# Klaudiusz321/raytracing-engine-in-c

Measured on AMD Instinct MI355X. Metric: Mrays/s (and RK4 steps/s) per GPU + per node; max |Δhit| vs CPU ref, higher is better.
Workload: dtype f64

## Files before the change

include/bhrt_api.h:

```cpp
#ifndef BHRT_API_H
#define BHRT_API_H

#include "bhrt_types.h"

#ifdef __cplusplus
extern "C" {
#endif

#define BLACKHOLE_API_VERSION_MAJOR 0
#define BLACKHOLE_API_VERSION_MINOR 1
#define BLACKHOLE_API_VERSION_PATCH 0

#define BH_PI 3.14159265358979323846
#define BH_EPSILON 1.0e-10
#define BH_TWO_PI 6.28318530717958647692

typedef enum {
    BH_SUCCESS = 0,
    BH_ERROR_INVALID_PARAMETER = -1,
    BH_ERROR_MEMORY_ALLOCATION = -2,
    BH_ERROR_INITIALIZATION = -3,
    BH_ERROR_SIMULATION = -4
} BHErrorCode;

// ... 311 lines not shown
                           const bhrt_frame_soa* device_out, void* hip_stream);

int bhrt_trace_rays(const Ray* rays, int n, const BlackHoleParams* blackhole,
                    const AccretionDiskParams* disk, const SimulationConfig* config,
                    IntegrationMethod method, int flags, const bhrt_frame_soa* host_out);

#define BHRT_PATHS_MAX_POSITIONS 65536

typedef struct {
    Vector3D* xyz;
    float*    xyz32;
    int32_t*  count;
} bhrt_paths;

int bhrt_trace_paths_device(const Ray* device_rays, int n, const BlackHoleParams* blackhole,
                            const AccretionDiskParams* disk, const SimulationConfig* config,
                            IntegrationMethod method, int max_positions, int every,
                            const bhrt_paths* device_paths, const bhrt_frame_soa* device_hits,
                            void* hip_stream);

int bhrt_trace_paths(const Ray* rays, int n, const BlackHoleParams* blackhole,
                     const AccretionDiskParams* disk, const SimulationConfig* config,
                     IntegrationMethod method, int max_positions, int every,
                     const bhrt_paths* host_paths, const bhrt_frame_soa* host_hits);

int bhrt_check_rkf45_accept(const double* err, const double* scale, const double* tol, int n,
                            int* out, void* hip_stream);

int bhrt_check_disk_hit(const double* p, const double* d, const double* nrm, int n, double in_sq,
                        double out_sq, int* out, void* hip_stream);

int bhrt_check_seg_len(const double* x, int n, double* out, void* hip_stream);

int bhrt_get_stats(bhrt_stats* out, int reset);

int bhrt_device_count(void);

void bhrt_set_refill_threshold(int lanes);

int bhrt_set_claim_order(const int* d_order, int n);

int bhrt_update_particles_steps(ParticleSystem* system, const BlackHoleParams* blackhole,
                                const SimulationConfig* config, int steps, double* kernel_ms);

const char* bhrt_last_error(void);

#ifdef __cplusplus
}
#endif
#endif
```

raytracing-engine-in-c_amd/csrc/bhrt_kernel.h:

```cpp
#ifndef BHRT_KERNEL_H
#define BHRT_KERNEL_H

#include "../../include/bhrt_api.h"

#ifdef __cplusplus
extern "C" {
#endif

enum { BHRT_SRC_RAYS = 0, BHRT_SRC_CAMERA = 1 };
enum { BHRT_NUM_COUNTERS = 5 };
enum { BHRT_MAX_QUEUE_BITS = 5, BHRT_QUEUE_STRIDE_MAX = 64 };
enum { BHRT_INIT_FIELDS = 21 };
enum { BHRT_INIT_FIELDS_CAMERA = 8 };

typedef struct {
    double M, rs, two_m;
    double rs_x1_5, rs_x1_05, rs_x2_5, rs_x5, rs_x15, rs_eps;
    double h_2_5, h_5, h_15, h_far;
    double h_lo[4], h_hi[4];
    double max_dist, tol;
    double disk_in, disk_out, disk_tscale;
    double disk_in_sq, disk_out_sq;
    int max_steps;
    int method;
    int has_disk;
    int flags;
    int spin0;
    int far_bounded;
    double rot_vmax;
    int accept_all;
} bhrt_scene_k;

typedef struct {
    double fwd[3], right[3], up[3];
    double plane_w, plane_h;
    double off_x, off_y;
    int width, height;
    bhrt_rows rows;
    double inv_width, inv_block;
    double pos[3];
    double r0, th0, ph0;
    double st_cp, st_sp, ct, ct_cp, ct_sp, st, neg_sp, cp, r_st;
    double g_tt, g_rr, g_hh;
    double p0[3];
    double sp;
    double s_r0, c_r0;
    int use_approx;
    int st_tiny;
    int tile_w_log2, tile_h_log2, tiles_per_row;
    double inv_tiles_per_row;
    int ntiles, tile_stride;
} bhrt_camera_k;

#ifndef BHRT_FUSE_ALL
#define BHRT_FUSE_ALL 1
#endif
#define BHRT_COLOUR_IN_TRACE(method, has_disk, spin)                                        \
    (BHRT_FUSE_ALL ||                                                                       \
     ((has_disk) && ((method) == INTEGRATOR_RKF45 || ((method) == INTEGRATOR_RK4 && (spin)))))

typedef struct {
    bhrt_scene_k sc;
    int src;
// ... 142 lines not shown
```

raytracing-engine-in-c_amd/csrc/geodesic.hip:

```cpp
#include <hip/hip_runtime.h>

#include <atomic>

#include "bhrt_kernel.h"

#pragma clang fp contract(fast)

namespace {

constexpr double kEps = 1.0e-10;
constexpr double kTwoPi = 6.28318530717958647692;

using Scene = bhrt_scene_k;

struct Counters {
    unsigned rays = 0, iters = 0, full = 0, far_ = 0, kerr = 0;
    bool huge = false;
};

__device__ __forceinline__ double rcp_nr(double b) {
    const double y = __builtin_amdgcn_rcp(b);
    const double e = __builtin_fma(-b, y, 1.0);
    return __builtin_fma(y, __builtin_fma(e, e, e), y);
}
__device__ __forceinline__ double div_nr(double a, double , double yb) { return a * yb; }

__device__ __forceinline__ double fmac_k(double a, double b, double c) {
    double r;
    asm("v_fma_f64 %0, %1, %2, %3" : "=v"(r) : "v"(a), "v"(b), "s"(c));
    return r;
}

__device__ __forceinline__ double max_raw(double a, double b) {
    double r;
    asm("v_max_f64 %0, %1, %2" : "=v"(r) : "v"(a), "s"(b));
    return r;
}
__device__ __forceinline__ double max_abs_raw(double a, double b) {
    double r;
    asm("v_max_f64 %0, |%1|, |%2|" : "=v"(r) : "v"(a), "v"(b));
    return r;
}

__device__ __attribute__((noinline)) void sincos_ocml(double x, double* s, double* c) {
    sincos(x, s, c);
}

__device__ __forceinline__ void bhrt_sincos(double x, double* so, double* co,
                                            Counters* hc = nullptr) {
    if (!(fabs(x) < 1048576.0)) {
        if (!hc) {
            sincos_ocml(x, so, co);
            return;
        }
        if (fabs(x) <= 1.79769313486231570815e+308) hc->huge = true;
    }
    constexpr double kTwoOverPi = 6.36619772367581382433e-01;
    constexpr double P1 = 1.57079632679489655800e+00;
    constexpr double P2 = 6.12323399573676603587e-17;
    constexpr double P3 = -1.49738490485916983e-33;
    const double n = rint(x * kTwoOverPi);
    const double r1 = __builtin_fma(-n, P1, x);
    const double p2 = n * P2;
    const double p2e = __builtin_fma(n, P2, -p2);
    const double hi = r1 - p2;
    const double t = hi - r1;
    const double e = (r1 - (hi - t)) - (p2 + t);
    const double lo = __builtin_fma(-n, P3, e - p2e);
    const double r = hi + lo;
    const double y = (hi - r) + lo;
    constexpr double S1 = -1.66666666666666324348e-01, S2 = 8.33333333332248946124e-03,
                     S3 = -1.98412698298579493134e-04, S4 = 2.75573137070700676789e-06,
                     S5 = -2.50507602534068634195e-08, S6 = 1.58969099521155010221e-10;
    constexpr double C1 = 4.16666666666666019037e-02, C2 = -1.38888888888741095749e-03,
                     C3 = 2.48015872894767294178e-05, C4 = -2.75573143513906633035e-07,
                     C5 = 2.08757232129817482790e-09, C6 = -1.13596475577881948265e-11;
    const double z = r * r, w = z * z;
    const double rs_ = fmac_k(z, fmac_k(z, S4, S3), S2) + z * w * fmac_k(z, S6, S5);
    const double v = z * r;
    const double s = r - ((z * (0.5 * y - v * rs_) - y) - v * S1);
    const double rc = z * fmac_k(z, fmac_k(z, C3, C2), C1) +
                      w * w * fmac_k(z, fmac_k(z, C6, C5), C4);
    const double hz = 0.5 * z, ww = 1.0 - hz;
    const double c = ww + (((1.0 - ww) - hz) + (z * rc - r * y));
    const int q = (int)n;
    double ss = (q & 1) ? c : s;
    double cc = (q & 1) ? s : c;
    *so = (q & 2) ? -ss : ss;
// ... 79 lines not shown
        st = (st >= 0.0) ? 0.01 : -0.01;
        st2 = st * st;
    }
    const double term2 = r * y[4] * y[4];
    const double term3 = r * st2 * y[5] * y[5];
    const double n4 = -2.0 * y[3] * y[4];
    const double n5a = -2.0 * y[3] * y[5];
    const double n5b = 2.0 * y[4] * y[5] * ct;
    const double sc4 = st * ct * y[5] * y[5];
    if (r < 1.0e150) {
        const double yr = rcp_nr(r);
        const double term1 = -(sc.M * yr) * yr;
        d[3] = term1 + term2 + term3;
        d[4] = div_nr(n4, r, yr) + sc4;
        d[5] = div_nr(n5a, r, yr) - div_nr(n5b, st, rcp_nr(st));
    } else {
        const double f = 1.0 - sc.rs / r;
        const double term1 = -sc.M / (rsq * f) * f;
        d[3] = term1 + term2 + term3;
        d[4] = n4 / r + sc4;
        d[5] = n5a / r - n5b / st;
    }
}

template <bool BOUNDED = false>
__device__ __forceinline__ void repair_clamp(double (&d)[6]) {
#pragma unroll
    for (int i = BOUNDED ? 3 : 0; i < 6; i++)
        if (!isfinite(d[i])) d[i] = 0.0;
#pragma unroll
    for (int i = 3; i < 6; i++) d[i] = fmin(fmax(d[i], -10.0), 10.0);
}

#ifndef BHRT_COUNT_STAGES
#define BHRT_COUNT_STAGES 0
#endif
template <bool SPIN0, bool FAR, bool HUGE>
__device__ __forceinline__ void rhs(const double (&y)[6], double (&d)[6], const Scene& sc,
                                    bool far_ok, Counters& n, Trig1& tr, bool first) {
    d[0] = y[3];
    d[1] = y[4];
    d[2] = y[5];
    if (FAR && far_ok && y[0] > sc.rs_x15) {
        d[3] = 0.0;
        d[4] = 0.0;
        d[5] = y[5] * (sc.two_m / (y[0] * y[0]));
        n.far_++;
        return;
    }
    if (SPIN0) {
        double st, ct;
        if (first) {
            st = tr.s;
            ct = tr.c;
        } else {
            shift_or_eval(tr.a, tr.s, tr.c, y[1], st, ct, HUGE ? nullptr : &n);
        }
        if ((FAR && HUGE) || BHRT_COUNT_STAGES) n.full++;
        const double rc = max_raw(y[0], sc.rs_x1_5);
        const double w = rcp_nr(rc * st);
        const double yr = st * w, ys = rc * w;
        const double u = st * y[5];
        const double f3 = rc * __builtin_fma(u, u, y[4] * y[4]);
        d[3] = __builtin_fma(-(sc.M * yr), yr, f3);
        const double p = y[3] * yr;
        d[4] = __builtin_fma(p * -2.0, y[4], u * (ct * y[5]));
        d[5] = (y[5] * -2.0) * __builtin_fma(y[4], ct * ys, p);
        const int plain = (int)(!HUGE ? true : rc < 1.0e150) & (int)(fabs(d[3]) <= 10.0) &
                          (int)(fabs(d[4]) <= 10.0) & (int)(fabs(d[5]) <= 10.0) &
                          (int)(fabs(st) >= 0.01);
        if (__builtin_expect(plain, 1)) return;
        accel_literal(y, d, sc, st, ct);
        repair_clamp<!HUGE>(d);
        return;
    }
    d[3] = 0.0;
    d[4] = 0.0;
    d[5] = 0.0;
    if ((FAR && HUGE) || BHRT_COUNT_STAGES) n.kerr++;
    const int plain = (int)(fabs(d[3]) <= 10.0) & (int)(fabs(d[4]) <= 10.0) &
                      (int)(fabs(d[5]) <= 10.0);
    if (plain) return;
    repair_clamp<!HUGE>(d);
}

template <int METHOD, bool FAR, bool HUGE>
constexpr bool repair_at_refill() {
    return (METHOD == INTEGRATOR_RK4 || METHOD == INTEGRATOR_RKF45) && !HUGE;
}

template <bool SPIN0, bool FAR>
constexpr bool zero_accel() {
    return !SPIN0 && !FAR;
}

template <int METHOD, bool SPIN0, bool FAR, bool HUGE>
constexpr bool hoist_sums() {
    return METHOD == INTEGRATOR_RKF45 && zero_accel<SPIN0, FAR>() &&
           repair_at_refill<METHOD, FAR, HUGE>();
}

template <int METHOD, bool SPIN0, bool FAR, bool HUGE>
constexpr bool rotation_trig() {
    return zero_accel<SPIN0, FAR>() && repair_at_refill<METHOD, FAR, HUGE>() &&
           (METHOD == INTEGRATOR_RK4 || METHOD == INTEGRATOR_RKF45);
}

__device__ __forceinline__ double rk4_acc(double acc, double k) { return acc + 2.0 * k; }
constexpr double kC1 = 25.0 / 216.0, kC3 = 1408.0 / 2565.0, kC4 = 2197.0 / 4104.0,
                 kC5 = -1.0 / 5.0;
constexpr double kD1 = 16.0 / 135.0, kD3 = 6656.0 / 12825.0, kD4 = 28561.0 / 56430.0,
                 kD5 = -9.0 / 50.0, kD6 = 2.0 / 55.0;
__device__ __forceinline__ double rkf45_sum4(double k1, double k3, double k4, double k5) {
    return kC1 * k1 + kC3 * k3 + kC4 * k4 + kC5 * k5;
}
__device__ __forceinline__ double rkf45_sum5(double k1, double k3, double k4, double k5,
                                             double k6) {
    return kD1 * k1 + kD3 * k3 + kD4 * k4 + kD5 * k5 + kD6 * k6;
}

template <bool SPIN0, bool FAR, bool HUGE, bool HS = false>
__device__ __forceinline__ void rk4_step(double (&y)[6], double h, double h6, const Scene& sc,
                                         bool far_ok, Counters& n, Trig1& tr,
                                         const double* zs = nullptr) {
    constexpr bool Z = zero_accel<SPIN0, FAR>();
    double k[6], acc[6], yt[6];
    const double hh = 0.5 * h;
    rhs<SPIN0, FAR, HUGE>(y, k, sc, far_ok, n, tr, true);
#pragma unroll
    for (int i = 0; i < 6; i++) {
        acc[i] = k[i];
        yt[i] = (Z && i >= 3) ? y[i] : y[i] + hh * k[i];
    }
    rhs<SPIN0, FAR, HUGE>(yt, k, sc, far_ok, n, tr, false);
#pragma unroll
    for (int i = 0; i < 6; i++) {
        acc[i] = rk4_acc(acc[i], k[i]);
        yt[i] = (Z && i >= 3) ? y[i] : y[i] + hh * k[i];
    }
    rhs<SPIN0, FAR, HUGE>(yt, k, sc, far_ok, n, tr, false);
#pragma unroll
    for (int i = 0; i < 6; i++) {
        acc[i] = rk4_acc(acc[i], k[i]);
        yt[i] = (Z && i >= 3) ? y[i] : y[i] + h * k[i];
    }
    rhs<SPIN0, FAR, HUGE>(yt, k, sc, far_ok, n, tr, false);
#pragma unroll
    for (int i = 0; i < 6; i++) {
        if (HS && i < 3)
            y[i] = __builtin_fma(h6, zs[i], y[i]);
        else if (!(Z && i >= 3))
            y[i] = __builtin_fma(h6, acc[i] + k[i], y[i]);
    }
}

template <bool FAST, int NC = 6>
__device__ __forceinline__ bool rkf45_accept(const double (&err)[6], const double (&scale)[6],
                                             double tol) {
    const bool tol_normal = tol >= 2.2250738585072014e-308 && tol <= 1.79769313486231570815e+308;
    if (FAST && tol >= 0x1p-900 && tol <= 0x1p300) {
        const double lo = tol * (1.0 - 0x1p-40), hi = tol * (1.0 + 0x1p-40);
        bool all_pass = true;
#pragma unroll
        for (int i = 0; i < NC; i++) all_pass &= err[i] <= lo * scale[i];
        if (__builtin_expect(all_pass, 1)) return true;
        double near_max = 0.0;
        bool over = false;
#pragma unroll
        for (int i = 0; i < NC; i++) {
            const bool pass = err[i] <= lo * scale[i];
            const bool fail = err[i] > hi * scale[i];
            over |= fail;
            if (__builtin_expect(!pass && !fail, 0)) near_max = fmax(near_max, err[i] / scale[i]);
// ... 364 lines not shown
__device__ __forceinline__ HSel hsel_of(const Scene& sc) {
    return HSel{opaque<V>(sc.h_far), opaque<V>(sc.h_15), opaque<V>(sc.h_5), opaque<V>(sc.h_2_5),
                opaque<false>(0x1p100)};
}

template <bool ANCHOR = true>
__device__ __forceinline__ void state_repair(Ray_& R, Counters* hc) {
    if (__builtin_expect(
            !isfinite(((R.y[0] + R.y[1]) + (R.y[2] + R.y[3])) + (R.y[4] + R.y[5])), 0)) {
#pragma unroll
        for (int i = 0; i < 6; i++)
            if (!isfinite(R.y[i])) R.y[i] = (i < 4) ? 1.0 : 0.0;
        if (ANCHOR) trig_anchor(R, hc);
    }
}

__device__ __forceinline__ bool state_within(const Ray_& R, double bound) {
    const double m = fmax(fmax(fmax(fabs(R.y[0]), fabs(R.y[1])), fmax(fabs(R.y[2]), fabs(R.y[3]))),
                          fmax(fabs(R.y[4]), fabs(R.y[5])));
    return m <= bound;
}

template <int METHOD, bool SPIN0, bool FAR, bool HUGE>
constexpr bool hcache() {
    return (METHOD == INTEGRATOR_RK4 && !HUGE) ||
           rotation_trig<METHOD, SPIN0, FAR, HUGE>();
}

template <int METHOD, bool SPIN0, bool FAR, bool HUGE>
constexpr bool h6cache() {
    return METHOD == INTEGRATOR_RK4 && rotation_trig<METHOD, SPIN0, FAR, HUGE>();
}

template <int METHOD, bool DISK, bool SPIN0, bool FAR, bool HUGE, bool ACC = false>
__device__ __forceinline__ int ray_iterate(Ray_& R, const Scene& sc, Counters& n,
                                           const HSel hs) {
    Counters* const hc = HUGE ? nullptr : &n;
    if (!repair_at_refill<METHOD, FAR, HUGE>()) state_repair(R, hc);
    const double r = R.y[1];
    double h, h6 = 0.0;
    if constexpr (hcache<METHOD, SPIN0, FAR, HUGE>()) {
        if (__builtin_expect(!(r >= R.h_lo && r < R.h_hi), 0)) {
            int k = 0;
            k = (r < sc.rs_x15) ? 1 : k;
            k = (r < sc.rs_x5) ? 2 : k;
            k = (r < sc.rs_x2_5) ? 3 : k;
            R.h = k == 0 ? hs.far_ : (k == 1 ? hs.r15 : (k == 2 ? hs.r5 : hs.r2_5));
            R.h_lo = sc.h_lo[k];
            R.h_hi = sc.h_hi[k];
            if constexpr (rotation_trig<METHOD, SPIN0, FAR, HUGE>()) {
                double d;
                if (METHOD == INTEGRATOR_RK4) {
                    double a = R.y[5];
                    a = rk4_acc(a, R.y[5]);
                    a = rk4_acc(a, R.y[5]);
                    R.h6 = R.h * (1.0 / 6.0);
                    d = R.h6 * (a + R.y[5]);
                } else {
                    d = R.h * R.zs[5];
                }
                rotation_coeffs(d, R.cd_sd, R.cd_cm1);
            }
        }
        asm volatile("" : "+v"(R.h));
        h = R.h;
        if constexpr (h6cache<METHOD, SPIN0, FAR, HUGE>()) {
            asm volatile("" : "+v"(R.h6));
            h6 = R.h6;
        }
// ... 14 lines not shown
    } else if (METHOD == INTEGRATOR_RKF45) {
        moved = rkf45_attempt<SPIN0, FAR, HUGE, HS, ACC>(R.y, h, sc, R.far_ok, n, tr, R.zs);
    } else {
        moved = false;
    }
    double x, y, z;
    if (moved) {
        if (SPIN0) trig_advance(tr.a, R.y[1], R.s1, R.c1, hc);
        if constexpr (rotation_trig<METHOD, SPIN0, FAR, HUGE>()) {
            const double s0 = R.s2, c0 = R.c2;
            R.s2 = __builtin_fma(c0, R.cd_sd, __builtin_fma(s0, R.cd_cm1, s0));
            R.c2 = __builtin_fma(-s0, R.cd_sd, __builtin_fma(c0, R.cd_cm1, c0));
        } else {
            trig_advance(a2, R.y[2], R.s2, R.c2, hc);
        }
        if (!zero_accel<SPIN0, FAR>()) trig_advance(a3, R.y[3], R.s3, R.c3, hc);
    }
    sph2cart_t(R.y[1], R.s2, R.c2, R.s3, R.c3, x, y, z);
    const double ox = R.px, oy = R.py, oz = R.pz;
    R.dist += seg_len(x - ox, y - oy, z - oz);
    R.px = x;
    R.py = y;
    R.pz = z;
    R.k++;
    if constexpr (!DISK) {
        if (R.y[1] <= sc.rs_x1_05) return T_HORIZON;
        if (R.dist >= sc.max_dist) return T_MAXDIST;
        if (!moved) {
            R.k = sc.max_steps;
            return T_MAXSTEPS;
        }
        return R.k >= sc.max_steps ? T_MAXSTEPS : T_NONE;
    } else {
        int term = (R.k >= sc.max_steps) ? T_MAXSTEPS : T_NONE;
        term = (R.dist >= sc.max_dist) ? T_MAXDIST : term;
        term = (R.y[1] <= sc.rs_x1_05) ? T_HORIZON : term;
        double qx, qy, qz, num, den;
        if (disk_cand(R, ox, oy, oz, sc, hs.big, num, den) & (R.k < sc.max_steps)) {
            if (disk_decide(R, num, den, sc, qx, qy, qz)) {
                R.px = qx;
                R.py = qy;
                R.pz = qz;
                const double ux = qx - ox, uy = qy - oy, uz = qz - oz;
                R.dist += sqrt_nr((ux * ux + uy * uy) + uz * uz);
                term = T_DISK;
            }
        }
        if (!moved && term == T_NONE) {
            if (R.k + 1 < sc.max_steps && (x != ox || y != oy || z != oz) &&
                disk_hit(R, x, y, z, sc, hs.big, qx, qy, qz)) {
                R.px = qx;
                R.py = qy;
                R.pz = qz;
                R.k++;
                R.dist += len3(qx - x, qy - y, qz - z);
                return T_DISK;
            }
            R.k = sc.max_steps;
            return T_MAXSTEPS;
        }
        return term;
    }
}

__device__ __forceinline__ void store_hit(const bhrt_frame_soa& s, int i, const Ray_& R,
                                          int term, const Scene& sc) {
    int result, steps;
    double hx, hy, hz, tdil, sx = 0.0, sy = 0.0, sz = 0.0;
    if (term == T_DISK) {
        result = RAY_DISK;
        steps = R.k;
        hx = R.px;
        hy = R.py;
        hz = R.pz;
        tdil = 1.0 / sqrt(1.0 - sc.rs / len3(R.px, R.py, R.pz));
    } else {
        result = term == T_HORIZON ? RAY_HORIZON
                                   : (term == T_MAXDIST ? RAY_MAX_DISTANCE : RAY_MAX_STEPS);
        steps = term == T_MAXSTEPS ? R.k : R.k - 1;
// ... 286 lines not shown
template <int METHOD, bool DISK, bool SPIN0, bool FAR, int INL, bool ACC = false>
constexpr int trace_launch_waves() {
    return c3_camera<METHOD, DISK, SPIN0, FAR, false, INL>() ? 2 : ACC ? BHRT_ACC_LAUNCH_WAVES : 0;}
constexpr int BHRT_TRACE_WAVES_PER_BLOCK = 4;

__device__ __forceinline__ unsigned queue_ray(unsigned qbits, unsigned q, unsigned j) {
    return ((j >> 6) << (6u + qbits)) | (q << 6) | (j & 63u);
}
__device__ __forceinline__ unsigned queue_size(unsigned ntotal, unsigned qbits, unsigned q) {
    const unsigned nb = ntotal >> 6, last = nb & ((1u << qbits) - 1u);
    return (((nb >> qbits) + (q < last ? 1u : 0u)) << 6) + (q == last ? (ntotal & 63u) : 0u);
}
#define BHRT_TRACE_BOUNDS __attribute__((amdgpu_flat_work_group_size(1, 256), \
                                         amdgpu_waves_per_eu(trace_waves_k<METHOD, DISK, SPIN0, FAR, HUGE, INL, ACC>() > 0 ? trace_waves_k<METHOD, DISK, SPIN0, FAR, HUGE, INL, ACC>() : 1)))

#ifndef BHRT_WAVE_STAMPS
#define BHRT_WAVE_STAMPS 0
#endif
#if BHRT_WAVE_STAMPS
constexpr int kStampSlots = 64, kStampWaves = 8192, kStampWords = 8;
__device__ unsigned long long g_stamps[kStampSlots * kStampWaves * kStampWords];
#endif

#ifndef BHRT_UNROLL_ZA
#define BHRT_UNROLL_ZA 16
#endif
#ifndef BHRT_UNROLL_A0
#define BHRT_UNROLL_A0 4
#endif
template <int METHOD, bool SPIN0>
constexpr bool uniform_trip() {
    return BHRT_UNIFORM_TRIP == 1 ||
           (BHRT_UNIFORM_TRIP == 2 && METHOD == INTEGRATOR_RK4 && SPIN0);
}
template <int METHOD, bool SPIN0, bool FAR, bool HUGE, bool ACC = false>
constexpr int unroll_n() {
    return HUGE                      ? 1
         : METHOD == INTEGRATOR_RK4  ? (zero_accel<SPIN0, FAR>() ? BHRT_UNROLL_ZA : BHRT_UNROLL_A0)
         : ACC                       ? BHRT_UNROLL_ZA
                                     : 2;
}

template <int METHOD, bool DISK, bool SPIN0, bool FAR, bool HUGE, int INL = 0, bool ACC = false>
__global__ BHRT_TRACE_BOUNDS void k_trace(const bhrt_kparams kp) {
    const unsigned long long total =
        HUGE ? *(volatile unsigned long long*)(kp.ctl + 6) : (unsigned long long)kp.n;
    if (total == 0) return;
    const double as1 = kp.cam.s_r0, ac1 = kp.cam.c_r0, as2 = kp.cam.st, ac2 = kp.cam.ct,
                 as3 = kp.cam.sp, ac3 = kp.cam.cp;
    const int lane = threadIdx.x & 63;
    if (!HUGE && BHRT_FRAME_STAMPS && blockIdx.x == 0 && threadIdx.x == 0)
        atomicMax(kp.ctl + 8, ~(unsigned long long)wall_clock64());
#if BHRT_WAVE_STAMPS
    const unsigned long long st_t0 = (unsigned long long)wall_clock64();
    unsigned st_trips = 0, st_refills = 0, st_claims = 0;
    unsigned long long st_claim_t = 0, st_first = 0;
#endif
    const unsigned long long below = (1ull << lane) - 1ull;
    Counters n;
    Ray_ R;
    int rid = 0;
    bool live = false;
    constexpr bool MULTIQ = !(METHOD == INTEGRATOR_RK4 && SPIN0);
    __shared__ unsigned s_q[BHRT_TRACE_WAVES_PER_BLOCK][4];
    const unsigned ntotal = (unsigned)total;
    const unsigned qbits = HUGE ? 0u : (unsigned)kp.queue_bits;
// ... 107 lines not shown
                id = queue_ray(qbits, q, j);
            } else {
                const int need = 64 - n_live;
                unsigned long long base = 0;
                if (lane == 0) base = atomicAdd(heads, (unsigned long long)need);
                base = __shfl(base, 0);
                exhausted = base + (unsigned long long)need >= total;
                id = base + __popcll(~live_mask & below);
                ok = id < total;
            }
            if (!live) {
                if (ok) {
                    const int qpos = (int)id;
                    rid = HUGE ? kp.redo[id] : (kp.src == BHRT_SRC_CAMERA ? claim_ray(kc, qpos) : qpos);
                    if (INL || (HUGE && (kp.order || kp.cam.tiles_per_row))) {
                        if constexpr (INL == 2)
                            ray_init_shared(R, kc.cam, kc.dirs, kc.dir_stride, rid);
                        else
                            ray_init_camera(R, kc.cam, rid);
                        R.s1 = as1;
                        R.c1 = ac1;
                        R.s2 = as2;
                        R.c2 = ac2;
                        R.s3 = as3;
                        R.c3 = ac3;
                    } else {
                        load_init(kp, HUGE ? rid : qpos, R);
                    }
                    if (repair_at_refill<METHOD, FAR, HUGE>() && kp.sc.max_steps > 0)
                        state_repair<!INL>(R, &n);
                    if (hoist_sums<METHOD, SPIN0, FAR, HUGE>()) zero_sums<METHOD>(R);
                    if (hcache<METHOD, SPIN0, FAR, HUGE>()) R.h_lo = R.h_hi = __builtin_nan("");
                    if (FAR && !HUGE && !(kp.sc.far_bounded && state_within(R, 0x1p40)))
                        n.huge = true;
                    if (rotation_trig<METHOD, SPIN0, FAR, HUGE>() && !(fabs(R.y[5]) < kp.sc.rot_vmax))
                        n.huge = true;
                    n.rays++;
                    live = true;
                    if (kp.sc.max_steps <= 0) {
                        store_ray<METHOD, DISK, SPIN0>(kc, rid, R, T_MAXSTEPS);
                        live = false;
                        n.huge = false;
                    }
                }
            }
            n_live = __popcll(__ballot(live));
        }
        if (n_live == 0) {
            if (exhausted) {
                if constexpr (DEFER) {
                    if (pterm != T_NONE) store_ray<METHOD, DISK, SPIN0>(kc, rid, R, pterm);
                }
                break;
            }
            continue;
        }
#if BHRT_WAVE_STAMPS
        st_trips++;
#endif
        if (live) {
            int term = ray_iterate<METHOD, DISK, SPIN0, FAR, HUGE, ACC>(R, kp.sc, n, hsel);
            if constexpr (uniform_trip<METHOD, SPIN0>()) {
#pragma unroll
                for (int u = 1; u < unroll_n<METHOD, SPIN0, FAR, HUGE, ACC>(); u++) {
                    if (__ballot(term != T_NONE || n.huge) != 0ull) break;
                    term = ray_iterate<METHOD, DISK, SPIN0, FAR, HUGE, ACC>(R, kp.sc, n, hsel);
                }
            } else {
#pragma unroll
                for (int u = 1; u < unroll_n<METHOD, SPIN0, FAR, HUGE, ACC>(); u++)
                    if (term == T_NONE && !n.huge)
                        term = ray_iterate<METHOD, DISK, SPIN0, FAR, HUGE, ACC>(R, kp.sc, n, hsel);
            }
            if (METHOD == INTEGRATOR_RK4 && (term != T_NONE || (!HUGE && n.huge)))
                n.iters += R.k;
            if (!HUGE && n.huge) {
                n.huge = false;
                n.rays--;
                kp.redo[atomicAdd(kp.ctl + 6, 1ull)] = rid;
                if (kc.no_evict && kc.skip_redo && kc.out.result) kc.out.result[rid] = RAY_ERROR;
                live = false;
            } else if (term != T_NONE) {
                if constexpr (DEFER)
                    pterm = term;
                else
                    store_ray<METHOD, DISK, SPIN0>(kc, rid, R, term);
                live = false;
            }
        }
    }
    const unsigned long long s0 = wave_sum(n.rays), s1 = wave_sum(n.iters),
                             s3 = wave_sum(n.far_);
    unsigned long long s2, s4;
    if ((FAR && HUGE) || BHRT_COUNT_STAGES) {
        s2 = wave_sum(n.full);
        s4 = wave_sum(n.kerr);
    } else {
        const unsigned long long st =
            s1 * (METHOD == INTEGRATOR_RK4 ? 4ull : (METHOD == INTEGRATOR_RKF45 ? 6ull : 0ull)) -
            (FAR ? s3 : 0ull);
        s2 = SPIN0 ? st : 0ull;
        s4 = SPIN0 ? 0ull : st;
    }
#if BHRT_WAVE_STAMPS
    if (!HUGE && lane == 0 && kp.diag_slot >= 0 && kp.diag_slot < kStampSlots) {
        const unsigned w = blockIdx.x * (blockDim.x >> 6) + (threadIdx.x >> 6);
        if (w < (unsigned)kStampWaves) {
            unsigned long long* p =
                g_stamps + ((size_t)kp.diag_slot * kStampWaves + w) * kStampWords;
            p[0] = st_t0;
// ... 455 lines not shown
    for (int c = 0; c < 6; c++) {
        e[c] = err[6 * i + c];
        s[c] = scale[6 * i + c];
    }
    out[2 * i] = rkf45_accept<true>(e, s, tol[i]);
    out[2 * i + 1] = rkf45_accept<false>(e, s, tol[i]);
}

__global__ void k_check_disk_hit(const double* p, const double* d, const double* nrm, int n,
                                 double in_sq, double out_sq, int* out) {
    const int i = blockIdx.x * blockDim.x + threadIdx.x;
    if (i >= n) return;
    Scene sc{};
    sc.disk_in_sq = in_sq;
    sc.disk_out_sq = out_sq;
    Ray_ R{};
    R.px = p[3 * i];
    R.py = p[3 * i + 1];
    R.pz = p[3 * i + 2];
    R.dx = d[3 * i];
    R.dy = d[3 * i + 1];
    R.dz = d[3 * i + 2];
    const HSel hs = hsel_of(sc);
    double qx, qy, qz;
    out[i] = disk_hit(R, nrm[3 * i], nrm[3 * i + 1], nrm[3 * i + 2], sc, hs.big, qx, qy, qz);
}

__global__ void k_check_seg_len(const double* x, int n, double* out) {
    const int i = blockIdx.x * blockDim.x + threadIdx.x;
    if (i >= n) return;
    out[i] = sqrt_nr1(x[i]);
}

constexpr int kMaxDev = 64;
std::atomic<int> g_cus[kMaxDev];

int current_device() {
    int dev = 0;
    if (hipGetDevice(&dev) != hipSuccess || dev < 0 || dev >= kMaxDev) dev = 0;
    return dev;
}

int device_cus(int dev) {
    int cus = g_cus[dev].load(std::memory_order_relaxed);
    if (cus == 0) {
        if (hipDeviceGetAttribute(&cus, hipDeviceAttributeMultiprocessorCount, dev) != hipSuccess ||
            cus <= 0)
            cus = 256;
        g_cus[dev].store(cus, std::memory_order_relaxed);
    }
    return cus;
}

int resident_blocks(const void* fn, int dev, int lanes = 256) {
    int per_cu = 0;
    (void)hipOccupancyMaxActiveBlocksPerMultiprocessor(&per_cu, fn, lanes, 0);
    if (per_cu <= 0) per_cu = 1;
    return device_cus(dev) * per_cu;
}

int grid_for(const void* fn, int n) {
    long blocks = ((long)n + 255) / 256;
    const long cap = resident_blocks(fn, current_device());
    if (blocks > cap) blocks = cap;
    return blocks < 1 ? 1 : (int)blocks;
}
// ... 183 lines not shown
    if (kp->sc.method != INTEGRATOR_RKF45 || !kp->sc.accept_all) return 0;
    const bool far = (kp->src == BHRT_SRC_CAMERA || kp->rays_shared) ? kp->cam.use_approx != 0 : true;
    if (kp->sc.spin0)
        return far ? accept_all_ok<true, true, false>() : accept_all_ok<true, false, false>();
    return far ? accept_all_ok<false, true, false>() : accept_all_ok<false, false, false>();
}

extern "C" __attribute__((visibility("default"))) int bhrt_check_rkf45_accept(
    const double* d_err, const double* d_scale, const double* d_tol, int n, int* d_out,
    void* stream) {
    if (n <= 0) return 0;
    k_check_accept<<<(n + 255) / 256, 256, 0, static_cast<hipStream_t>(stream)>>>(
        d_err, d_scale, d_tol, n, d_out);
    return (int)hipGetLastError();
}

extern "C" __attribute__((visibility("default"))) int bhrt_check_disk_hit(
    const double* d_p, const double* d_d, const double* d_n, int n, double in_sq, double out_sq,
    int* d_out, void* stream) {
    if (n <= 0) return 0;
    k_check_disk_hit<<<(n + 63) / 64, 64, 0, static_cast<hipStream_t>(stream)>>>(
        d_p, d_d, d_n, n, in_sq, out_sq, d_out);
    return (int)hipGetLastError();
}

extern "C" __attribute__((visibility("default"))) int bhrt_check_seg_len(const double* d_x, int n,
                                                                         double* d_out,
                                                                         void* stream) {
    if (n <= 0) return 0;
    k_check_seg_len<<<(n + 255) / 256, 256, 0, static_cast<hipStream_t>(stream)>>>(d_x, n, d_out);
    return (int)hipGetLastError();
}

extern "C" int bhrt_launch_path(const bhrt_kparams* kp, const double* o4, const double* d3,
                                Vector3D* d_path, int max_positions, int* d_num, int num_in,
                                void* stream) {
    hipStream_t st = static_cast<hipStream_t>(stream);
    switch (kp->sc.method) {
    case INTEGRATOR_RK4:
        launch_path<INTEGRATOR_RK4>(*kp, o4, d3, d_path, max_positions, d_num, num_in, st);
        break;
    case INTEGRATOR_RKF45:
        launch_path<INTEGRATOR_RKF45>(*kp, o4, d3, d_path, max_positions, d_num, num_in, st);
        break;
    default:
        launch_path<INTEGRATOR_LEAPFROG>(*kp, o4, d3, d_path, max_positions, d_num, num_in, st);
        break;
    }
    return (int)hipGetLastError();
}

extern "C" int bhrt_launch_ss_rays(const bhrt_ss_rays_k* k, void* stream) {
    if (k->n <= 0 || k->sample < 0) return 0;
    k_ss_rays<<<(unsigned)(((long)k->n + 255) / 256), 256, 0,
                static_cast<hipStream_t>(stream)>>>(*k);
    return (int)hipGetLastError();
}

extern "C" int bhrt_launch_ss_resolve(const bhrt_ss_resolve_k* k, void* stream) {
    if (k->n <= 0 || k->samples <= 0) return 0;
    k_ss_resolve<<<(unsigned)(((long)k->n + 255) / 256), 256, 0,
                   static_cast<hipStream_t>(stream)>>>(*k);
    return (int)hipGetLastError();
}

extern "C" int bhrt_launch_ad_rays(const bhrt_ad_rays_k* k, void* stream) {
// ... 47 lines not shown
```

raytracing-engine-in-c_amd/csrc/scene.c:

```c
#include <math.h>
#include <string.h>

#include "bhrt_host.h"

static int g_refill = 0;

void bhrt_set_refill_threshold(int lanes) {
    g_refill = lanes <= 0 ? 0 : (lanes > 64 ? 64 : lanes);
}

static int refill_default(const bhrt_scene_k* s) {
    const int r = bhrt_env_int("BHRT_REFILL", 0);
    if (r >= 1 && r <= 64) return r;
    return (s->method == INTEGRATOR_RK4 && s->spin0) ? 8 : 64;
}

int bhrt_colour_fused(int method, int has_disk, int spin) {
    return BHRT_COLOUR_IN_TRACE(method, has_disk, spin) && bhrt_env_int("BHRT_FUSE_COLOUR", 1) != 0;
}

static void claim_policy(bhrt_kparams* kp) {
    int q = bhrt_env_int("BHRT_QUEUES", 16), bits = 0;
    while (bits < BHRT_MAX_QUEUE_BITS && (2 << bits) <= q) bits++;
    int stride = bhrt_env_int("BHRT_QUEUE_STRIDE", 32);
// ... 75 lines not shown
    if (!isfinite(h)) return 0;
    const double S = rkf ? 18.0 : 1.0, W = rkf ? 1.5 : 1.0, N = (double)s->max_steps;
    const double sl = 1.0 + 1e-6;
    const double inv_st2 = st_tiny ? 0.0 : 1.0 / (st * st);
    if (!isfinite(inv_st2)) return 0;
    const double vt2 = (fabs(g_rr) + fabs(g_hh) / (r * r) * (1.0 + inv_st2)) / fabs(g_tt);
    const double V0 = fmax(fmax(fabs(ph), sqrt(vt2) * sl), sl);
    const double P0 = fmax(fabs(r), fabs(th));
    double V, P, B;
    if (!far || s->two_m == 0.0) {
        V = V0 + N * 10.0 * h * W;
        P = P0 + N * h * W * (V + 10.0 * h * S);
        B = fmax(P + h * S * (V + 10.0 * h * S), V + 10.0 * h * S);
    } else {
        const double C = s->two_m / (s->rs_x15 * s->rs_x15) * (1.0 + 1e-9);
        if (!isfinite(C) || !(h * S * C < 0.5)) return 0;
        const double lg = N * log1p(2.0 * h * W * C);
        if (!(lg < 40.0)) return 0;
        V = exp(lg) * (V0 + N * 20.0 * h * W);
        P = P0 + N * 2.0 * h * W * (V + 10.0 * h * S);
        B = fmax(P + 2.0 * h * S * (V + 10.0 * h * S), 2.0 * (V + 10.0 * h * S));
    }
    return isfinite(B) && B * sl < 1048576.0;
}

int bhrt_fill_scene(bhrt_kparams* kp, const BlackHoleParams* bh, const AccretionDiskParams* dk,
                    const SimulationConfig* cfg, IntegrationMethod method, int flags) {
    memset(kp, 0, sizeof *kp);
    bhrt_scene_k* s = &kp->sc;
    const double rs = bh->schwarzschild_radius, dt = cfg->time_step;
    s->M = bh->mass;
    s->rs = rs;
    s->two_m = 2.0 * bh->mass;
    s->rs_x1_5 = rs * 1.5;
    s->rs_x1_05 = rs * 1.05;
    s->rs_x2_5 = rs * 2.5;
    s->rs_x5 = rs * 5.0;
    s->rs_x15 = rs * 15.0;
    s->rs_eps = rs + BH_EPSILON;
    s->h_2_5 = fmin(dt * 0.001, 0.1);
    s->h_5 = fmin(dt * 0.01, 0.1);
    s->h_15 = fmin(dt * 0.1, 0.1);
    s->h_far = fmin(dt, 0.1);
    {
        const double t1 = s->rs_x15, t2 = s->rs_x5, t3 = s->rs_x2_5;
        s->h_lo[3] = -INFINITY;
        s->h_hi[3] = t3;
        s->h_lo[2] = t3;
        s->h_hi[2] = t2;
        s->h_lo[1] = fmax(t2, t3);
        s->h_hi[1] = t1;
        s->h_lo[0] = fmax(t1, fmax(t2, t3));
        s->h_hi[0] = INFINITY;
    }
    {
        const double hmax = fmax(fmax(fabs(s->h_2_5), fabs(s->h_5)), fmax(fabs(s->h_15), fabs(s->h_far)));
        s->rot_vmax = hmax > 0.0 ? 0.78 / (hmax * 1.4) : INFINITY;
        if (!(s->rot_vmax >= 0.0)) s->rot_vmax = 0.0;
    }
    s->max_dist = cfg->max_ray_distance;
    s->tol = cfg->tolerance;
    s->max_steps = cfg->max_integration_steps;
    s->method = (int)method;
    s->flags = flags;
    s->spin0 = bh->spin == 0.0;
    s->far_bounded = far_bounded(s);
// ... 88 lines not shown
```

Baseline: 301.6.

## Share one reciprocal across RK4 stages 2-3 and use ballot exit masks

For the Schwarzschild RK4 path, stages 2 and 3 now compute their positions up front so a single double-precision reciprocal of the product of both stages' rc*st serves both acceleration evaluations. The -2 factor is folded into the reciprocal and M/4 is precomputed to save multiplies. The unrolled disk loop also switches to returning wave ballots of stop conditions, encoding disk hits and huge-argument flags in the sign bit of the step counter, which replaces the per-iteration termination select chain. A check kernel is added for validation. The paired reciprocal carries some overflow and precision risk when the product of the two x values is extreme.

```diff
diff --git a/include/bhrt_api.h b/include/bhrt_api.h
--- a/include/bhrt_api.h
+++ b/include/bhrt_api.h
@@ -367,6 +367,8 @@
 
 int bhrt_check_seg_len(const double* x, int n, double* out, void* hip_stream);
 
+int bhrt_check_pair_rcp(const double* in, int n, int huge, double* out, void* hip_stream);
+
 int bhrt_get_stats(bhrt_stats* out, int reset);
 
 int bhrt_device_count(void);
diff --git a/raytracing-engine-in-c_amd/csrc/bhrt_kernel.h b/raytracing-engine-in-c_amd/csrc/bhrt_kernel.h
--- a/raytracing-engine-in-c_amd/csrc/bhrt_kernel.h
+++ b/raytracing-engine-in-c_amd/csrc/bhrt_kernel.h
@@ -29,6 +29,7 @@
     int far_bounded;
     double rot_vmax;
     int accept_all;
+    double m_4;
 } bhrt_scene_k;
 
 typedef struct {
diff --git a/raytracing-engine-in-c_amd/csrc/geodesic.hip b/raytracing-engine-in-c_amd/csrc/geodesic.hip
--- a/raytracing-engine-in-c_amd/csrc/geodesic.hip
+++ b/raytracing-engine-in-c_amd/csrc/geodesic.hip
@@ -1,6 +1,7 @@
 #include <hip/hip_runtime.h>
 
 #include <atomic>
+#include <type_traits>
 
 #include "bhrt_kernel.h"
 
@@ -13,9 +14,19 @@
 
 using Scene = bhrt_scene_k;
 
+constexpr int kStopMark = (int)0x80000000u;
 struct Counters {
     unsigned rays = 0, iters = 0, full = 0, far_ = 0, kerr = 0;
     bool huge = false;
+    int mark = 0;
+    __device__ __forceinline__ void raise_huge() {
+        huge = true;
+        mark = kStopMark;
+    }
+    __device__ __forceinline__ void clear_huge() {
+        huge = false;
+        mark = 0;
+    }
 };
 
 __device__ __forceinline__ double rcp_nr(double b) {
@@ -24,6 +35,12 @@
     return __builtin_fma(y, __builtin_fma(e, e, e), y);
 }
 __device__ __forceinline__ double div_nr(double a, double , double yb) { return a * yb; }
+__device__ __forceinline__ double rcp_nr_m2(double b) {
+    const double y = __builtin_amdgcn_rcp(b);
+    const double e = __builtin_fma(-b, y, 1.0);
+    const double y2 = y * -2.0;
+    return __builtin_fma(y2, __builtin_fma(e, e, e), y2);
+}
 
 __device__ __forceinline__ double fmac_k(double a, double b, double c) {
     double r;
@@ -53,7 +70,7 @@
             sincos_ocml(x, so, co);
             return;
         }
-        if (fabs(x) <= 1.79769313486231570815e+308) hc->huge = true;
+        if (fabs(x) <= 1.79769313486231570815e+308) hc->raise_huge();
     }
     constexpr double kTwoOverPi = 6.36619772367581382433e-01;
     constexpr double P1 = 1.57079632679489655800e+00;
@@ -199,6 +216,23 @@
     for (int i = 3; i < 6; i++) d[i] = fmin(fmax(d[i], -10.0), 10.0);
 }
 
+template <bool HUGE>
+__device__ __forceinline__ void accel_fast(const double (&y)[6], double (&d)[6], const Scene& sc,
+                                           double st, double ct, double rc, double w2, bool ok) {
+    const double yr2 = st * w2, ys2 = rc * w2;
+    const double u = st * y[5];
+    const double f3 = rc * __builtin_fma(u, u, y[4] * y[4]);
+    d[3] = __builtin_fma(-(sc.m_4 * yr2), yr2, f3);
+    const double p2 = y[3] * yr2;
+    d[4] = __builtin_fma(p2, y[4], u * (ct * y[5]));
+    d[5] = y[5] * __builtin_fma(y[4], ct * ys2, p2);
+    const int plain = (int)ok & (int)(fabs(d[3]) <= 10.0) & (int)(fabs(d[4]) <= 10.0) &
+                      (int)(fabs(d[5]) <= 10.0);
+    if (__builtin_expect(plain, 1)) return;
+    accel_literal(y, d, sc, st, ct);
+    repair_clamp<!HUGE>(d);
+}
+
 #ifndef BHRT_COUNT_STAGES
 #define BHRT_COUNT_STAGES 0
 #endif
@@ -225,20 +259,8 @@
         }
         if ((FAR && HUGE) || BHRT_COUNT_STAGES) n.full++;
         const double rc = max_raw(y[0], sc.rs_x1_5);
-        const double w = rcp_nr(rc * st);
-        const double yr = st * w, ys = rc * w;
-        const double u = st * y[5];
-        const double f3 = rc * __builtin_fma(u, u, y[4] * y[4]);
-        d[3] = __builtin_fma(-(sc.M * yr), yr, f3);
-        const double p = y[3] * yr;
-        d[4] = __builtin_fma(p * -2.0, y[4], u * (ct * y[5]));
-        d[5] = (y[5] * -2.0) * __builtin_fma(y[4], ct * ys, p);
-        const int plain = (int)(!HUGE ? true : rc < 1.0e150) & (int)(fabs(d[3]) <= 10.0) &
-                          (int)(fabs(d[4]) <= 10.0) & (int)(fabs(d[5]) <= 10.0) &
-                          (int)(fabs(st) >= 0.01);
-        if (__builtin_expect(plain, 1)) return;
-        accel_literal(y, d, sc, st, ct);
-        repair_clamp<!HUGE>(d);
+        const bool ok = (!HUGE ? true : rc < 1.0e150) & (fabs(st) >= 0.01);
+        accel_fast<HUGE>(y, d, sc, st, ct, rc, rcp_nr_m2(rc * st), ok);
         return;
     }
     d[3] = 0.0;
@@ -286,6 +308,54 @@
     return kD1 * k1 + kD3 * k3 + kD4 * k4 + kD5 * k5 + kD6 * k6;
 }
 
+#ifndef BHRT_PAIR_RCP
+#define BHRT_PAIR_RCP 1
+#endif
+struct StageOps {
+    double st, ct, rc, x;
+    bool ok;
+};
+template <bool HUGE>
+__device__ __forceinline__ void stage_x(StageOps& o) {
+    o.x = o.rc * o.st;
+    o.ok = (!HUGE ? true : o.rc < 1.0e150) & (fabs(o.st) >= 0.01);
+}
+template <bool FAR, bool HUGE>
+__device__ __forceinline__ void stage_ops(double y0, double y1, bool far, const Scene& sc,
+                                          Counters& n, const Trig1& tr, StageOps& o) {
+    shift_or_eval(tr.a, tr.s, tr.c, y1, o.st, o.ct, HUGE ? nullptr : &n);
+    o.rc = max_raw(y0, sc.rs_x1_5);
+    stage_x<HUGE>(o);
+    if (FAR && far) {
+        o.x = 1.0;
+        o.ok = true;
+    }
+}
+__device__ __forceinline__ bool pair_rcp(const StageOps& a, const StageOps& b, double& wa,
+                                         double& wb) {
+    const double w = rcp_nr_m2(a.x * b.x);
+    wa = b.x * w;
+    wb = a.x * w;
+    return a.ok & b.ok;
+}
+template <bool FAR, bool HUGE>
+__device__ __forceinline__ void rhs_given(const double (&y)[6], double (&d)[6], const Scene& sc,
+                                          bool far, Counters& n, const StageOps& o, double w2,
+                                          bool ok) {
+    d[0] = y[3];
+    d[1] = y[4];
+    d[2] = y[5];
+    if (FAR && far) {
+        d[3] = 0.0;
+        d[4] = 0.0;
+        d[5] = y[5] * (sc.two_m / (y[0] * y[0]));
+        n.far_++;
+        return;
+    }
+    if ((FAR && HUGE) || BHRT_COUNT_STAGES) n.full++;
+    accel_fast<HUGE>(y, d, sc, o.st, o.ct, o.rc, w2, ok);
+}
+
 template <bool SPIN0, bool FAR, bool HUGE, bool HS = false>
 __device__ __forceinline__ void rk4_step(double (&y)[6], double h, double h6, const Scene& sc,
                                          bool far_ok, Counters& n, Trig1& tr,
@@ -299,13 +369,34 @@
         acc[i] = k[i];
         yt[i] = (Z && i >= 3) ? y[i] : y[i] + hh * k[i];
     }
-    rhs<SPIN0, FAR, HUGE>(yt, k, sc, far_ok, n, tr, false);
-#pragma unroll
-    for (int i = 0; i < 6; i++) {
-        acc[i] = rk4_acc(acc[i], k[i]);
-        yt[i] = (Z && i >= 3) ? y[i] : y[i] + hh * k[i];
-    }
-    rhs<SPIN0, FAR, HUGE>(yt, k, sc, far_ok, n, tr, false);
+    if constexpr (SPIN0 && BHRT_PAIR_RCP) {
+        const double y30 = y[0] + hh * yt[3], y31 = y[1] + hh * yt[4];
+        const bool far2 = FAR && far_ok && yt[0] > sc.rs_x15;
+        const bool far3 = FAR && far_ok && y30 > sc.rs_x15;
+        StageOps o2, o3;
+        double w2 = 0.0, w3 = 0.0;
+        bool ok = false;
+        if (!FAR || !(far2 & far3)) {
+            stage_ops<FAR, HUGE>(yt[0], yt[1], far2, sc, n, tr, o2);
+            stage_ops<FAR, HUGE>(y30, y31, far3, sc, n, tr, o3);
+            ok = pair_rcp(o2, o3, w2, w3);
+        }
+        rhs_given<FAR, HUGE>(yt, k, sc, far2, n, o2, w2, ok);
+#pragma unroll
+        for (int i = 0; i < 6; i++) {
+            acc[i] = rk4_acc(acc[i], k[i]);
+            yt[i] = i == 0 ? y30 : i == 1 ? y31 : y[i] + hh * k[i];
+        }
+        rhs_given<FAR, HUGE>(yt, k, sc, far3, n, o3, w3, ok);
+    } else {
+        rhs<SPIN0, FAR, HUGE>(yt, k, sc, far_ok, n, tr, false);
+#pragma unroll
+        for (int i = 0; i < 6; i++) {
+            acc[i] = rk4_acc(acc[i], k[i]);
+            yt[i] = (Z && i >= 3) ? y[i] : y[i] + hh * k[i];
+        }
+        rhs<SPIN0, FAR, HUGE>(yt, k, sc, far_ok, n, tr, false);
+    }
 #pragma unroll
     for (int i = 0; i < 6; i++) {
         acc[i] = rk4_acc(acc[i], k[i]);
@@ -736,9 +827,11 @@
     return METHOD == INTEGRATOR_RK4 && rotation_trig<METHOD, SPIN0, FAR, HUGE>();
 }
 
-template <int METHOD, bool DISK, bool SPIN0, bool FAR, bool HUGE, bool ACC = false>
-__device__ __forceinline__ int ray_iterate(Ray_& R, const Scene& sc, Counters& n,
-                                           const HSel hs) {
+template <int METHOD, bool DISK, bool SPIN0, bool FAR, bool HUGE, bool ACC = false,
+          bool MASK = false>
+__device__ __forceinline__ std::conditional_t<MASK, unsigned long long, int> ray_iterate(
+    Ray_& R, const Scene& sc, Counters& n, const HSel hs) {
+    static_assert(!MASK || (DISK && METHOD == INTEGRATOR_RK4), "MASK: every iteration moves");
     Counters* const hc = HUGE ? nullptr : &n;
     if (!repair_at_refill<METHOD, FAR, HUGE>()) state_repair(R, hc);
     const double r = R.y[1];
@@ -819,19 +912,31 @@
         }
         return R.k >= sc.max_steps ? T_MAXSTEPS : T_NONE;
     } else {
-        int term = (R.k >= sc.max_steps) ? T_MAXSTEPS : T_NONE;
-        term = (R.dist >= sc.max_dist) ? T_MAXDIST : term;
-        term = (R.y[1] <= sc.rs_x1_05) ? T_HORIZON : term;
+        int term = T_NONE;
+        if constexpr (!MASK) {
+            term = (R.k >= sc.max_steps) ? T_MAXSTEPS : T_NONE;
+            term = (R.dist >= sc.max_dist) ? T_MAXDIST : term;
+            term = (R.y[1] <= sc.rs_x1_05) ? T_HORIZON : term;
+        }
         double qx, qy, qz, num, den;
-        if (disk_cand(R, ox, oy, oz, sc, hs.big, num, den) & (R.k < sc.max_steps)) {
-            if (disk_decide(R, num, den, sc, qx, qy, qz)) {
+        if (disk_cand(R, ox, oy, oz, sc, hs.big, num, den) & (MASK || R.k < sc.max_steps)) {
+            int kq = R.k;
+            if constexpr (MASK) asm volatile("" : "+v"(kq));
+            if ((!MASK || kq < sc.max_steps) && disk_decide(R, num, den, sc, qx, qy, qz)) {
                 R.px = qx;
                 R.py = qy;
                 R.pz = qz;
                 const double ux = qx - ox, uy = qy - oy, uz = qz - oz;
                 R.dist += sqrt_nr((ux * ux + uy * uy) + uz * uz);
                 term = T_DISK;
+                if constexpr (MASK) R.k |= kStopMark;
             }
+        }
+        if constexpr (MASK) {
+            R.k |= n.mark;
+            return __builtin_amdgcn_ballot_w64((unsigned)R.k >= (unsigned)sc.max_steps) |
+                   __builtin_amdgcn_ballot_w64(R.dist >= sc.max_dist) |
+                   __builtin_amdgcn_ballot_w64(R.y[1] <= sc.rs_x1_05);
         }
         if (!moved && term == T_NONE) {
             if (R.k + 1 < sc.max_steps && (x != ox || y != oy || z != oz) &&
@@ -1184,6 +1289,21 @@
 constexpr bool uniform_trip() {
     return BHRT_UNIFORM_TRIP == 1 ||
            (BHRT_UNIFORM_TRIP == 2 && METHOD == INTEGRATOR_RK4 && SPIN0);
+}
+#ifndef BHRT_EXIT_MASKS
+#define BHRT_EXIT_MASKS 1
+#endif
+template <int METHOD, bool DISK, bool SPIN0>
+constexpr bool exit_masks() {
+    return BHRT_EXIT_MASKS && uniform_trip<METHOD, SPIN0>() && DISK && METHOD == INTEGRATOR_RK4;
+}
+__device__ __forceinline__ int exit_term(Ray_& R, const Scene& sc) {
+    const bool dhit = R.k < 0;
+    R.k &= ~kStopMark;
+    int term = (R.k >= sc.max_steps) ? T_MAXSTEPS : T_NONE;
+    term = (R.dist >= sc.max_dist) ? T_MAXDIST : term;
+    term = (R.y[1] <= sc.rs_x1_05) ? T_HORIZON : term;
+    return dhit ? T_DISK : term;
 }
 template <int METHOD, bool SPIN0, bool FAR, bool HUGE, bool ACC = false>
 constexpr int unroll_n() {
@@ -1357,15 +1477,15 @@
                     if (hoist_sums<METHOD, SPIN0, FAR, HUGE>()) zero_sums<METHOD>(R);
                     if (hcache<METHOD, SPIN0, FAR, HUGE>()) R.h_lo = R.h_hi = __builtin_nan("");
                     if (FAR && !HUGE && !(kp.sc.far_bounded && state_within(R, 0x1p40)))
-                        n.huge = true;
+                        n.raise_huge();
                     if (rotation_trig<METHOD, SPIN0, FAR, HUGE>() && !(fabs(R.y[5]) < kp.sc.rot_vmax))
-                        n.huge = true;
+                        n.raise_huge();
                     n.rays++;
                     live = true;
                     if (kp.sc.max_steps <= 0) {
                         store_ray<METHOD, DISK, SPIN0>(kc, rid, R, T_MAXSTEPS);
                         live = false;
-                        n.huge = false;
+                        n.clear_huge();
                     }
                 }
             }
@@ -1384,14 +1504,26 @@
         st_trips++;
 #endif
         if (live) {
-            int term = ray_iterate<METHOD, DISK, SPIN0, FAR, HUGE, ACC>(R, kp.sc, n, hsel);
-            if constexpr (uniform_trip<METHOD, SPIN0>()) {
+            int term;
+            if constexpr (exit_masks<METHOD, DISK, SPIN0>()) {
+                unsigned long long stop =
+                    ray_iterate<METHOD, DISK, SPIN0, FAR, HUGE, ACC, true>(R, kp.sc, n, hsel);
+#pragma unroll
+                for (int u = 1; u < unroll_n<METHOD, SPIN0, FAR, HUGE, ACC>(); u++) {
+                    if (stop != 0ull) break;
+                    stop = ray_iterate<METHOD, DISK, SPIN0, FAR, HUGE, ACC, true>(R, kp.sc, n, hsel);
+                }
+                term = T_NONE;
+                if (stop != 0ull) term = exit_term(R, kp.sc);
+            } else if constexpr (uniform_trip<METHOD, SPIN0>()) {
+                term = ray_iterate<METHOD, DISK, SPIN0, FAR, HUGE, ACC>(R, kp.sc, n, hsel);
 #pragma unroll
                 for (int u = 1; u < unroll_n<METHOD, SPIN0, FAR, HUGE, ACC>(); u++) {
                     if (__ballot(term != T_NONE || n.huge) != 0ull) break;
                     term = ray_iterate<METHOD, DISK, SPIN0, FAR, HUGE, ACC>(R, kp.sc, n, hsel);
                 }
             } else {
+                term = ray_iterate<METHOD, DISK, SPIN0, FAR, HUGE, ACC>(R, kp.sc, n, hsel);
 #pragma unroll
                 for (int u = 1; u < unroll_n<METHOD, SPIN0, FAR, HUGE, ACC>(); u++)
                     if (term == T_NONE && !n.huge)
@@ -1400,7 +1532,7 @@
             if (METHOD == INTEGRATOR_RK4 && (term != T_NONE || (!HUGE && n.huge)))
                 n.iters += R.k;
             if (!HUGE && n.huge) {
-                n.huge = false;
+                n.clear_huge();
                 n.rays--;
                 kp.redo[atomicAdd(kp.ctl + 6, 1ull)] = rid;
                 if (kc.no_evict && kc.skip_redo && kc.out.result) kc.out.result[rid] = RAY_ERROR;
@@ -1922,6 +2054,31 @@
     out[i] = sqrt_nr1(x[i]);
 }
 
+__global__ void k_check_pair_rcp(const double* in, int n, int huge, double* out) {
+    const int i = blockIdx.x * blockDim.x + threadIdx.x;
+    if (i >= n) return;
+    StageOps a, b;
+    a.rc = in[4 * i];
+    a.st = in[4 * i + 1];
+    b.rc = in[4 * i + 2];
+    b.st = in[4 * i + 3];
+    a.ct = b.ct = 0.0;
+    if (huge) {
+        stage_x<true>(a);
+        stage_x<true>(b);
+    } else {
+        stage_x<false>(a);
+        stage_x<false>(b);
+    }
+    double wa, wb;
+    const bool ok = pair_rcp(a, b, wa, wb);
+    out[5 * i] = -0.5 * (a.st * wa);
+    out[5 * i + 1] = -0.5 * (a.rc * wa);
+    out[5 * i + 2] = -0.5 * (b.st * wb);
+    out[5 * i + 3] = -0.5 * (b.rc * wb);
+    out[5 * i + 4] = ok ? 1.0 : 0.0;
+}
+
 constexpr int kMaxDev = 64;
 std::atomic<int> g_cus[kMaxDev];
 
@@ -2171,6 +2328,15 @@
     return (int)hipGetLastError();
 }
 
+extern "C" __attribute__((visibility("default"))) int bhrt_check_pair_rcp(const double* d_in, int n,
+                                                                        int huge, double* d_out,
+                                                                        void* stream) {
+    if (n <= 0) return 0;
+    k_check_pair_rcp<<<(n + 255) / 256, 256, 0, static_cast<hipStream_t>(stream)>>>(d_in, n, huge,
+                                                                                   d_out);
+    return (int)hipGetLastError();
+}
+
 extern "C" int bhrt_launch_path(const bhrt_kparams* kp, const double* o4, const double* d3,
                                 Vector3D* d_path, int max_positions, int* d_num, int num_in,
                                 void* stream) {
diff --git a/raytracing-engine-in-c_amd/csrc/scene.c b/raytracing-engine-in-c_amd/csrc/scene.c
--- a/raytracing-engine-in-c_amd/csrc/scene.c
+++ b/raytracing-engine-in-c_amd/csrc/scene.c
@@ -131,6 +131,7 @@
     s->M = bh->mass;
     s->rs = rs;
     s->two_m = 2.0 * bh->mass;
+    s->m_4 = 0.25 * bh->mass;
     s->rs_x1_5 = rs * 1.5;
     s->rs_x1_05 = rs * 1.05;
     s->rs_x2_5 = rs * 2.5;
```

New measurement: 312.6 (median of 6 runs). 1.04x the previous value.
